# pbalcer/libpga

Measured on AMD Instinct MI355X. Metric: generations/sec + evals/sec, OneMax pop=1M 1024-bit, 1/2/4/8 MI355X, higher is better.
Workload: dtype u1-bitpacked; 1 GPU; model=OneMax-1024bit, global_batch=1048576, seq_len=1024, parallelism=island1, pop_per_gpu=1048576, selection=tournament-2, crossover=uniform, mutation=bit_flip, elitism=1, topology=ring, device=AMD Radeon Graphics

## Files before the change

csrc/include/pga/binary_dev.hpp:

```cpp
#pragma once
#include <hip/hip_runtime.h>

#include <type_traits>

#include "pga/device.hpp"
#include "pga/ops.hpp"
#include "pga/tp.hpp"

typedef __attribute__((address_space(3))) const unsigned int* pga_lds_words;
extern "C" __device__ float pga_user_objective(pga_lds_words words, unsigned int nbits, const float* data);

namespace pga {
#ifdef PGA_JIT_GEN
namespace jitgen {
#else
namespace {
#endif

using namespace dev;


template <int OBJ>
struct BinObj {
  uint32_t u = 0;
  uint32_t first0 = 0xFFFFFFFFu;
  float v = 0.f, w = 0.f;

  __device__ __forceinline__ void add(const GenArgs& a, uint4 x, uint32_t c) {
    const uint32_t wd[4] = {x.x, x.y, x.z, x.w};
    if (OBJ == OBJ_ONEMAX) {
      u += __popc(x.x) + __popc(x.y) + __popc(x.z) + __popc(x.w);
    } else if (OBJ == OBJ_KNAPSACK) {
      const float* val = a.obj_data;
      const float* wt = a.obj_data + a.L;
#pragma unroll
      for (int j = 0; j < 4; ++j) {
        uint32_t bits = wd[j];
        const uint32_t base = c * 128u + 32u * j;
        while (bits) {
          uint32_t b = __ffs(bits) - 1;
          bits &= bits - 1;
          v += val[base + b];
          w += wt[base + b];
        }
      }
    } else if (OBJ == OBJ_TRAP) {
      const uint32_t k = (uint32_t)a.obj_i;
      const uint32_t km = k >= 32 ? 0xFFFFFFFFu : ((1u << k) - 1u);
#pragma unroll
      for (int j = 0; j < 4; ++j) {
        const uint32_t base = c * 128u + 32u * j;
        for (uint32_t i = 0; i < 32u; i += k) {
          if (base + i + k > a.L) break;
          uint32_t ones = __popc((wd[j] >> i) & km);
          u += ones == k ? k : (k - 1 - ones);
        }
      }
    } else if (OBJ == OBJ_LEADING_ONES) {
#pragma unroll
      for (int j = 0; j < 4; ++j) {
        uint32_t inv = ~wd[j];
        if (inv != 0u) {
          uint32_t p = c * 128u + 32u * j + (__ffs(inv) - 1);
          first0 = p < first0 ? p : first0;
          break;
        }
      }
    }
  }

  template <int GS>
  __device__ __forceinline__ float finish(const GenArgs& a) {
    if (OBJ == OBJ_ONEMAX || OBJ == OBJ_TRAP) return (float)group_sum_u<GS>(u);
    if (OBJ == OBJ_KNAPSACK) {
      float vv = group_sum<GS>(v), ww = group_sum<GS>(w);
      return ww <= a.obj_f0 ? vv : a.obj_f0 - ww;
    }
    if (OBJ == OBJ_LEADING_ONES) {
      uint32_t m = group_min_u<GS>(first0);
      return (float)(m < a.L ? m : a.L);
    }
    return 0.f;
  }
};

__device__ __forceinline__ uint4 u4(u32x4 v) { return make_uint4(v.x, v.y, v.z, v.w); }
__device__ __forceinline__ uint4 and4(uint4 a, uint4 b) { return make_uint4(a.x & b.x, a.y & b.y, a.z & b.z, a.w & b.w); }
__device__ __forceinline__ uint4 xor4(uint4 a, uint4 b) { return make_uint4(a.x ^ b.x, a.y ^ b.y, a.z ^ b.z, a.w ^ b.w); }
__device__ __forceinline__ uint4 mix4(uint4 a, uint4 b, uint4 m) {
  return make_uint4((a.x & m.x) | (b.x & ~m.x), (a.y & m.y) | (b.y & ~m.y), (a.z & m.z) | (b.z & ~m.z),
                    (a.w & m.w) | (b.w & ~m.w));
}
__device__ __forceinline__ uint4 range_keep_a(uint32_t c, uint32_t lo, uint32_t hi) {
  const uint32_t b0 = c * 128u;
  return make_uint4(~range_mask32(b0, lo, hi), ~range_mask32(b0 + 32, lo, hi), ~range_mask32(b0 + 64, lo, hi),
                    ~range_mask32(b0 + 96, lo, hi));
}
__device__ __forceinline__ uint4 bit4(uint32_t b) {
  const uint32_t m = 1u << (b & 31u), j = b >> 5;
  return make_uint4(j == 0 ? m : 0u, j == 1 ? m : 0u, j == 2 ? m : 0u, j == 3 ? m : 0u);
}
__device__ __forceinline__ uint32_t chunk_len(uint32_t L, uint32_t c) {
  const uint32_t b = c * 128u;
  return L - b >= 128u ? 128u : L - b;
}

typedef int v4i __attribute__((ext_vector_type(4)));
constexpr int kObjKnapMfma = 1000;
constexpr uint32_t kKnapSlices = 8;
constexpr uint32_t kKnapMaxCols = 16;

__device__ __forceinline__ v4i expand16(uint32_t h) {
  v4i r;
  r[0] = (int)(__umul24(h & 0xFu, 0x00204081u) & 0x01010101u);
  r[1] = (int)(__umul24((h >> 4) & 0xFu, 0x00204081u) & 0x01010101u);
  r[2] = (int)(__umul24((h >> 8) & 0xFu, 0x00204081u) & 0x01010101u);
  r[3] = (int)(__umul24((h >> 12) & 0xFu, 0x00204081u) & 0x01010101u);
  return r;
}

__device__ __forceinline__ uint32_t knap_slot(uint32_t m, uint32_t h) { return 4u * m + (h ^ ((m >> 1) & 3u)); }
constexpr uint32_t kKnapCStride = 20;
constexpr uint32_t kKnapScratch = 16 * kKnapCStride / 4;

template <int GS>
__device__ __forceinline__ float knap_mfma(const GenArgs& a, uint4 v, uint32_t lane, uint32_t q, uint4* scr,
                                           const uint4* tab) {
  constexpr uint32_t R = GS / 4;
  const uint32_t D = a.knap_dig, NC = a.knap_cols;
  scr[knap_slot(lane >> 2, lane & 3u)] = v;
  wave_lds_sync();
  const uint32_t h = lane >> 4, n = lane & 15u;
  const uint4 x = scr[knap_slot(n, h)];
  const uint32_t xs[4] = {x.x, x.y, x.z, x.w};
  const uint4* tb = tab + h * kKnapMaxCols + n;
  v4i acc = {0, 0, 0, 0};
#pragma unroll
  for (uint32_t s = 0; s < kKnapSlices; ++s) {
    const uint4 t = tb[s * 4u * kKnapMaxCols];
    const uint32_t bits = (s & 1u) ? (xs[s >> 1] >> 16) : (xs[s >> 1] & 0xFFFFu);
    acc = __builtin_amdgcn_mfma_i32_16x16x64_i8(expand16(bits), v4i{(int)t.x, (int)t.y, (int)t.z, (int)t.w}, acc,
                                                0, 0, 0);
  }
  wave_lds_sync();
  int* cl = (int*)scr;
  *(v4i*)(cl + n * kKnapCStride + 4u * h) = acc;
  wave_lds_sync();
  const uint32_t g = lane / GS;
  uint32_t V = 0, W = 0;
  for (uint32_t e = q; e < NC; e += GS) {
    const uint32_t r = e / (2u * D), d = e % D;
    const uint32_t c = (uint32_t)cl[e * kKnapCStride + g * R + r] << (8u * d);
    if ((e / D) & 1u) W += c;
    else V += c;
  }
  const float vv = (float)(int)group_sum_u<GS>(V), ww = (float)(int)group_sum_u<GS>(W);
  return ww <= a.obj_f0 ? vv : a.obj_f0 - ww;
}

template <int GS, bool NH = false>
__device__ __forceinline__ uint4 sparse_continue(const GenArgs& a, uint64_t child, uint32_t K, uint32_t n, uint32_t j,
                                              uint4 fm, uint32_t q, uint32_t gbase) {
  u32x4 blk = draw<NH>(a.key, ST_BMUT, child, j >> 2);
  while (n < K) {
    if ((j & 3u) == 0u) blk = draw<NH>(a.key, ST_BMUT, child, j >> 2);
    const uint32_t p = word_to_index(sel4(blk, j & 3u), a.L);
    ++j;
    const uint32_t b = p & 127u;
    const bool own = (p >> 7) == q;
    const uint32_t wd = sel4(u32x4{fm.x, fm.y, fm.z, fm.w}, b >> 5);
    unsigned long long bal = __ballot(own && ((wd >> (b & 31u)) & 1u));
    if (GS < 64) bal = (bal >> gbase) & ((1ull << GS) - 1ull);
    if (bal == 0ull) {
      if (own) fm = xor4(fm, bit4(b));
      ++n;
    }
  }
  return fm;
}

template <bool NH>
__device__ __forceinline__ uint4 sparse_seq(const RngKey& key, uint64_t child, uint32_t kk, uint32_t L, uint32_t& jn) {
  uint32_t w0 = 0xFFFFFFFFu, w1 = 0xFFFFFFFFu, w2 = 0xFFFFFFFFu, w3 = 0xFFFFFFFFu;
  uint32_t n = 0, j = 0;
  u32x4 blk{0, 0, 0, 0};
  while (n < kk) {
    if ((j & 3u) == 0u) blk = draw<NH>(key, ST_BMUT, child, j >> 2);
    const uint32_t p = word_to_index(sel4(blk, j & 3u), L);
    ++j;
    const bool seen = (w0 & 0xFFFFu) == p || (w0 >> 16) == p || (w1 & 0xFFFFu) == p || (w1 >> 16) == p ||
                      (w2 & 0xFFFFu) == p || (w2 >> 16) == p || (w3 & 0xFFFFu) == p || (w3 >> 16) == p;
    if (!seen) {
      const uint32_t sh = (n & 1u) * 16u, keep = ~(0xFFFFu << sh), v = p << sh, wi = n >> 1;
      w0 = wi == 0u ? (w0 & keep) | v : w0;
      w1 = wi == 1u ? (w1 & keep) | v : w1;
      w2 = wi == 2u ? (w2 & keep) | v : w2;
      w3 = wi == 3u ? (w3 & keep) | v : w3;
      ++n;
    }
  }
  jn = j;
  return make_uint4(w0, w1, w2, w3);
}

template <int GS, int OBJ, int MODE>
__global__ __launch_bounds__(kBlock) void binary_kernel(GenArgs a, unsigned long long* best_parts) {
  resolve_gen(a);
  __shared__ unsigned long long lds_red[kBlock / 64];
  __shared__ uint32_t lds_elite;
  __shared__ uint32_t lds_thr[kMutCap];

  const uint32_t lane = lane_id();
  const uint32_t q = lane & (GS - 1);
  const uint32_t gbase = lane & ~(uint32_t)(GS - 1);
  constexpr uint32_t GPB = kBlock / GS;
  const uint32_t g_in_block = threadIdx.x / GS;
  const uint64_t rs = a.row_words >> 2;
  const uint4* cur = (const uint4*)a.cur;
  uint4* nxt = (uint4*)a.next;
  const uint32_t nchunks = a.chunks;
  const uint32_t L = a.L;
  constexpr bool MUTATES = MODE == MODE_GEN || MODE == MODE_MUTATE;
  constexpr bool EVALS = OBJ != OBJ_NONE && (MODE == MODE_GEN || MODE == MODE_INIT || MODE == MODE_EVAL);
  const bool bitflip = MUTATES && a.mutation == MUT_BIT_FLIP && a.mut_rate > 0.f;
  const bool sparse = bitflip && a.mut_sparse;
  const bool reset_one = MUTATES && a.mutation == MUT_RESET_ONE;

  if (MODE == MODE_GEN && a.n_elite > 0 && a.elite_idx == nullptr && blockIdx.x == 0) {
    unsigned long long b = block_reduce_parts(a.best_cur, a.n_best_cur, lds_red);
    if (threadIdx.x == 0) lds_elite = (uint32_t)best_index(b);
  }
  if (bitflip)
    for (uint32_t i = threadIdx.x; i < kMutCap; i += kBlock) lds_thr[i] = a.mut_thr[i];
  __syncthreads();

  unsigned long long my_best = 0;
  ScoreStats st;
  const uint64_t stride = (uint64_t)gridDim.x * GPB;
  for (uint64_t child = (uint64_t)blockIdx.x * GPB + g_in_block; child < a.S; child += stride) {
    float score = 0.f;
    {
      const bool elite = MODE == MODE_GEN && child < a.n_elite;
      uint32_t pa = 0, pb = 0;
      bool xo = false;
      uint32_t blo = 0, bhi = 0;
      u32x4 misc{0, 0, 0, 0};
      if (MODE == MODE_GEN || MODE == MODE_CROSS || MODE == MODE_MUTATE) misc = bin_misc(a.key, child);
      if (elite) {
        pa = pb = a.elite_idx ? a.elite_idx[child] : lds_elite;
      } else if (MODE == MODE_GEN || MODE == MODE_CROSS) {
        st_select_parents(a, child, pa, pb);
        xo = a.crossover != XO_NONE && do_crossover(a, misc.x);
        if (a.crossover == XO_ONE_POINT) {
          blo = word_to_index(misc.y, L);
          bhi = L;
        } else if (a.crossover == XO_TWO_POINT) {
          uint32_t c1 = word_to_index(misc.y, L);
          uint32_t c2 = word_to_index(misc.z, L);
          blo = c1 < c2 ? c1 : c2;
          bhi = c1 < c2 ? c2 : c1;
        }
      }
      uint32_t rpos = 0xFFFFFFFFu;
      if (reset_one && !elite && misc.w < a.mut_ind_thresh) rpos = word_to_index(bin_mut_word(a.key, child, 0), L);
      uint4 fm = make_uint4(0, 0, 0, 0);
      if (sparse && !elite) fm = sparse_continue<GS>(a, child, binom_count(misc.w, lds_thr), 0, 0, fm, q, gbase);

      BinObj<OBJ> acc;
      for (uint32_t c0 = 0; c0 < nchunks; c0 += GS) {
        const uint32_t c = c0 + q;
        if (c >= nchunks) continue;
        uint4 v = make_uint4(0, 0, 0, 0);
        if (MODE == MODE_INIT) {
          v = u4(draw(a.key, ST_INIT, child, c));
        } else if (MODE == MODE_EVAL || MODE == MODE_MUTATE) {
          v = cur[child * rs + c];
        } else {
          const uint4 A = cur[(uint64_t)pa * rs + c];
          if (xo) {
            const uint4 B = cur[(uint64_t)pb * rs + c];
            const uint4 m = a.crossover == XO_UNIFORM ? u4(draw(a.key, ST_XO, child, c)) : range_keep_a(c, blo, bhi);
            v = mix4(A, B, m);
          } else {
            v = A;
          }
        }
        if (c == nchunks - 1) v = and4(v, u4(a.last_mask));
        if (bitflip && !sparse && !elite) {
          v = xor4(v, u4(chunk_flip_mask(a, child, c, chunk_len(L, c), bin_chunk_mut_word(a.key, child, c), lds_thr)));
        } else if (sparse) {
          v = xor4(v, fm);
        } else if (reset_one && (rpos >> 7) == c) {
          v = xor4(v, bit4(rpos & 127u));
        }
        if (MODE != MODE_EVAL) nxt[child * rs + c] = v;
        if (EVALS) acc.add(a, v, c);
      }
      if (EVALS) score = acc.template finish<GS>(a);
    }
    if (EVALS && q == 0) {
      a.score_next[child] = score;
      if (a.key_next) a.key_next[child] = (uint16_t)score;
      const unsigned long long pb = pack_best(score, child);
      my_best = pb > my_best ? pb : my_best;
      st.add(score);
    }
  }
  if (EVALS && best_parts) {
    unsigned long long b = block_max_u64(my_best, lds_red);
    if (threadIdx.x == 0) best_parts[blockIdx.x] = b;
    if (a.stats_parts) block_stats_store(st, a.stats_parts);
  }
}


#ifdef PGA_TP_TIMING
__device__ unsigned long long pga_tp_clk[kMaxGrid * 4][8];
#endif


__device__ __forceinline__ uint32_t pos16(uint4 r1, uint32_t k) {
  const uint32_t w = sel4(u32x4{r1.x, r1.y, r1.z, r1.w}, k >> 1);
  return (k & 1u) ? (w >> 16) : (w & 0xFFFFu);
}

template <int GS, int OBJ, bool FULL, bool DENSE>
__device__ __forceinline__ void binary_gen_tp_body(GenArgs a, unsigned long long* best_parts) {
  resolve_gen(a);
  const uint32_t NW = blockDim.x >> 6;
  constexpr uint32_t NG = 64 / GS;
  constexpr uint32_t PD = tp_prefetch_depth(GS);
  constexpr bool EVALS = OBJ != OBJ_NONE;
  constexpr bool KEY = OBJ == OBJ_ONEMAX || OBJ == OBJ_LEADING_ONES || OBJ == OBJ_TRAP;
  uint4(*lds_rec)[2][64][2] = (uint4(*)[2][64][2])pga_dyn_lds;
  uint2* lds_par = (uint2*)(pga_dyn_lds + NW * 4096u);
  __shared__ uint32_t lds_thr[kMutCap];
  __shared__ uint32_t lds_el[kTpMaxElite];
  __shared__ unsigned long long lds_red[kTpMaxWaves];
  __shared__ uint32_t lds_next;
  __shared__ uint32_t lds_tnext;
  __shared__ uint32_t lds_ready[kTpMaxSegs];
  constexpr bool KMF = OBJ == kObjKnapMfma;
  __shared__ uint4 lds_kscr[KMF ? kTpMaxWaves : 1][kKnapScratch];
  __shared__ uint4 lds_ktab[KMF ? kKnapSlices * 4 * kKnapMaxCols : 1];
  constexpr bool JIT = OBJ == kObjJit;
  constexpr bool HISTK = KEY && !JIT;

  const uint32_t lane = lane_id(), wid = threadIdx.x >> 6;
  const uint32_t q = lane & (GS - 1), gbase = lane & ~(uint32_t)(GS - 1), g = lane / GS;
  const uint4* cur = (const uint4*)a.cur;
  uint4* nxt = (uint4*)a.next;
  const uint32_t L = a.L, S = (uint32_t)a.S;
  const bool have = FULL || q < a.chunks, last = q == a.chunks - 1;
  const uint32_t qq = have ? q : 0u;
  const uint32_t clen = have ? chunk_len(L, q) : 0u;
  const bool xo_on = a.crossover != XO_NONE;
  const bool range = a.crossover != XO_UNIFORM;
  const bool bitflip = a.mutation == MUT_BIT_FLIP && a.mut_rate > 0.f;
  const bool sparse = !DENSE && bitflip;
  const bool reset_one = !DENSE && a.mutation == MUT_RESET_ONE;
  const uint4 lmask = u4(a.last_mask);
  const uint32_t rb = a.row_words * 4u;
#define ELEM(T, base, i) (*(T*)((char*)(base) + (uint32_t)(i) * (uint32_t)sizeof(T)))
#define ROW(base, row, ch) (*(uint4*)((char*)(base) + ((uint32_t)(row) * rb + (uint32_t)(ch) * 16u)))

  const uint32_t U = tp_unit(a, NG);
  const uint32_t nst = U / NG;
  uint32_t bbegin, bend;
  tp_block_range(S, U, bbegin, bend, a.tp_skew);
  const uint32_t pcap = tp_par_cap(NW);
  uint4* lds_stage = (uint4*)(pga_dyn_lds + NW * 4096u + pcap * 8u) + wid * (kJitStageSteps * 64u);
  (void)lds_stage;
  uint32_t* lds_hist = (uint32_t*)(pga_dyn_lds + NW * 4096u + pcap * 8u);
  const bool hist = HISTK && (a.key_hist != nullptr || a.rank_counts != nullptr);
  const uint32_t hmax = a.hist_bins - 1u;

  __shared__ uint32_t lds_pro;
  bool pro_ok = false;
  if (KMF)
    for (uint32_t i = threadIdx.x; i < kKnapSlices * 4 * kKnapMaxCols; i += blockDim.x)
      lds_ktab[i] = ((const uint4*)a.knap_tab)[i];
  if (threadIdx.x == 0) lds_next = lds_tnext = lds_pro = 0;
  if (threadIdx.x < kTpMaxSegs) lds_ready[threadIdx.x] = 0;
  if (hist) {
    for (uint32_t i = threadIdx.x; i < a.hist_bins; i += blockDim.x) lds_hist[i] = 0;
    if (a.hist_zero)
      for (uint32_t i = blockIdx.x * blockDim.x + threadIdx.x; i < a.hist_zero_words; i += gridDim.x * blockDim.x)
        a.hist_zero[i] = 0;
  }

  unsigned long long my_best = 0;
  ScoreStats st;
  uint4(*rec)[64][2] = lds_rec[wid];
  static_assert(sizeof(lds_rec[0]) >= kSegBatches * 64 * sizeof(uint4), "contestant staging");
#ifdef PGA_TP_TIMING
  const unsigned long long clk0 = clock64(), rt0 = wall_clock64();
  unsigned long long clk_t = 0, clk_b = 0, n_bred = 0, clk_spin = 0;
#endif
  for (uint32_t rbeg = bbegin; rbeg < bend; rbeg += pcap) {
    const uint32_t rend = rbeg + pcap < bend ? rbeg + pcap : bend;
    const uint32_t nu = (rend - rbeg + U - 1) / U;
    const uint32_t nseg = (rend - rbeg + kSegBatches * 64 - 1) / (kSegBatches * 64);
    __syncthreads();
#ifdef PGA_TP_TIMING
    const unsigned long long clkA = clock64();
#endif
    if (rbeg == bbegin && wid == 0) {
      if (a.n_elite > 0 && bbegin < a.n_elite) {
        if (a.elite_idx) {
          for (uint32_t i = lane; i < a.n_elite; i += 64) lds_el[i] = a.elite_idx[i];
        } else {
          const unsigned long long b = wave_reduce_parts(a.best_cur, a.n_best_cur);
          if (lane == 0) lds_el[0] = (uint32_t)best_index(b);
        }
      }
      if (bitflip)
        for (uint32_t i = lane; i < kMutCap; i += 64) lds_thr[i] = a.mut_thr[i];
      __builtin_amdgcn_fence(__ATOMIC_RELEASE, "workgroup");
      tp_flag_set(&lds_pro);
    }

    for (;;) {
      const uint32_t sg = tp_ticket(&lds_tnext, lane);
      if (sg >= nseg) break;
      const uint32_t begin = rbeg + sg * kSegBatches * 64u;
      const uint32_t end = begin + kSegBatches * 64u < rend ? begin + kSegBatches * 64u : rend;
      uint2* par = lds_par + sg * kSegBatches * 64u;
      tp_select_segment<KEY ? TP_KEY16 : TP_F32>(a, begin, end, lane, &rec[0][0][0], par);
      __builtin_amdgcn_fence(__ATOMIC_RELEASE, "workgroup");
      tp_flag_set(&lds_ready[sg]);
    }
    if (NW < kTpMaxWaves) __syncthreads();
#ifdef PGA_TP_TIMING
    const unsigned long long clkB = clock64();
    clk_t += clkB - clkA;
#endif

#ifdef PGA_TP_TIMING
#define PGA_TP_SPIN0 const unsigned long long sp0_ = clock64();
#define PGA_TP_SPIN1 clk_spin += clock64() - sp0_;
#else
#define PGA_TP_SPIN0
#define PGA_TP_SPIN1
#endif
#define PGA_TP_RESOLVE(US, UE, SL)                                                                              \
  {                                                                                                             \
    if (!pro_ok) {                                           \
      while (__hip_atomic_load(&lds_pro, __ATOMIC_RELAXED, __HIP_MEMORY_SCOPE_WORKGROUP) == 0u)                 \
        __builtin_amdgcn_s_sleep(1);                                                                            \
      __builtin_amdgcn_fence(__ATOMIC_ACQUIRE, "workgroup");                                                    \
      pro_ok = true;                                                                                            \
    }                                                                                                           \
    const uint32_t tc = (US) + lane;                                                                            \
    const uint32_t cc = tc < (UE) ? tc : (UE) - 1;                                                              \
                                                             \
    const uint32_t sg_ = ((US) - rbeg) / (kSegBatches * 64u);                                                   \
    PGA_TP_SPIN0                                                                                                \
    while (__hip_atomic_load(&lds_ready[sg_], __ATOMIC_RELAXED, __HIP_MEMORY_SCOPE_WORKGROUP) == 0u)            \
      __builtin_amdgcn_s_sleep(1);                                                                              \
    PGA_TP_SPIN1                                                                                                \
    __builtin_amdgcn_fence(__ATOMIC_ACQUIRE, "workgroup");                                                      \
    const uint2 pp = lds_par[cc - rbeg];                              \
    uint32_t pa = pp.x, pb = pp.y;                                                                              \
    const u32x4 misc = bin_misc<true>(a.key, cc);                                                               \
    const bool elite = tc < a.n_elite;                                                                          \
    const bool xo = !elite && xo_on && do_crossover(a, misc.x);                                                 \
    if (elite) pa = lds_el[tc];                                                                                 \
    pb = xo ? pb : pa;                                                                                          \
    uint32_t lo = 0, hi = 0;                                                                                    \
    if (range && xo) {                                                                                          \
      const uint32_t x1 = word_to_index(misc.y, L);                                                             \
      if (a.crossover == XO_ONE_POINT) {                                                                        \
        lo = x1;                                                                                                \
        hi = L;                                                                                                 \
      } else {                                                                                                  \
        const uint32_t x2 = word_to_index(misc.z, L);                                                           \
        lo = x1 < x2 ? x1 : x2;                                                                                 \
        hi = x1 < x2 ? x2 : x1;                                                                                 \
      }                                                                                                         \
    }                                                                                                           \
    uint32_t K = 0, jn = 0;                                                                                     \
    uint4 P = make_uint4(0xFFFFFFFFu, 0xFFFFFFFFu, 0xFFFFFFFFu, 0xFFFFFFFFu);                                   \
    if (reset_one && !elite && misc.w < a.mut_ind_thresh) {                                                     \
      K = 1;                                                                                                    \
      P.x = word_to_index(bin_mut_word<true>(a.key, cc, 0), L) | 0xFFFF0000u;                                   \
    }                                                                                                           \
    if (sparse && !elite) {                                                                                     \
      K = binom_count(misc.w, lds_thr);                                                                         \
      if (K > 0u) {                                                                                             \
        const uint32_t kk = K < kRecPos ? K : kRecPos;                                                          \
        const u32x4 m0 = draw<true>(a.key, ST_BMUT, cc, 0);                                                     \
        const uint32_t c0 = word_to_index(m0.x, L), c1 = word_to_index(m0.y, L);                                \
        const uint32_t c2 = word_to_index(m0.z, L), c3 = word_to_index(m0.w, L);                                \
                              \
        const bool slow = kk > 4u || (kk > 1u && c0 == c1) || (kk > 2u && (c2 == c0 || c2 == c1)) ||            \
                          (kk > 3u && (c3 == c0 || c3 == c1 || c3 == c2));                                      \
        P = make_uint4(c0 | (c1 << 16), c2 | (c3 << 16), 0xFFFFFFFFu, 0xFFFFFFFFu);                             \
        jn = kk;                                                                                                \
        if (slow) P = sparse_seq<true>(a.key, cc, kk, L, jn);                                                   \
      }                                                                                                         \
    }                                                                                                           \
    const uint32_t meta = (K > 255u ? 255u : K) | ((jn > 0xFFFFu ? 0xFFFFu : jn) << 8) | (elite ? 1u << 31 : 0u); \
    uint4(*r)[2] = rec[(SL)];                                                                                   \
    r[lane][0] = make_uint4(pa, pb, lo | (hi << 16), meta);                                                     \
    r[lane][1] = P;                                                                                             \
  }

    constexpr uint32_t kNoUnit = 0xFFFFFFFFu;
#define PGA_TP_NEXT(US, UE)                                                                                 \
  {                                                                                                         \
    US = kNoUnit;                                                                                           \
    const uint32_t tk_ = tp_ticket(&lds_next, lane);                                                        \
    if (tk_ < nu) {                                                                                         \
      US = rbeg + tk_ * U;                                                                                  \
      UE = US + U < rend ? US + U : rend;                                                                   \
    }                                                                                                       \
  }

    uint32_t ns, ne = 0;
    PGA_TP_NEXT(ns, ne)
    if (ns != kNoUnit) {
      uint32_t slot = 0, i = 0, bs = ns, be = ne;
      PGA_TP_NEXT(ns, ne)
      PGA_TP_RESOLVE(bs, be, 0u)
      uint32_t lslot = 0, li = 0, lbs = bs, lbe = be;
      bool lpend = false, lmore = true, done = false;

#define PGA_TP_LOAD(YA, YB)                                                                                 \
  {                                                                                                         \
    if (lpend) {                                                                \
      PGA_TP_RESOLVE(ns, ne, lslot ^ 1u)                                                                    \
      lslot ^= 1u;                                                                                          \
      li = 0;                                                                                               \
      lbs = ns;                                                                                             \
      lbe = ne;                                                                                             \
      lpend = false;                                                                                        \
      PGA_TP_NEXT(ns, ne)                                                                                   \
    }                                                                                                       \
    const uint4 r = rec[lmore ? lslot : slot][(lmore ? li : i) * NG + g][0];                                \
    YA = ROW(cur, r.x, qq);                                                                                 \
    YB = ROW(cur, r.y, qq);                                                                                 \
    if (lmore && ++li == nst) {                                                                             \
      lpend = ns != kNoUnit;                                                                                \
      lmore = lpend;                                                                                        \
    }                                                                                                       \
  }

#define PGA_TP_STEP(XA, XB, YA, YB)                                                                         \
  {                                                                                                         \
    PGA_TP_LOAD(YA, YB)                                                                                     \
    const uint32_t c = bs + i * NG + g;                                                                     \
    const uint4 r0 = rec[slot][i * NG + g][0];                                                              \
    const uint32_t meta = r0.w;                                                                             \
    const uint4 m = range ? range_keep_a(q, r0.z & 0xFFFFu, r0.z >> 16) : u4(draw<true>(a.key, ST_XO, c, q)); \
    uint4 v = mix4(XA, XB, m);                                                                              \
    if (last) v = and4(v, lmask);                                                                           \
    uint4 fm = make_uint4(0, 0, 0, 0);                                                                      \
    if (DENSE) {                                                                                            \
      if (bitflip && !(meta >> 31))                                            \
        fm = u4(chunk_flip_mask(a, c, q, clen, bin_chunk_mut_word<true>(a.key, c, q), lds_thr));            \
    } else {                                                                                                \
      const uint32_t K = meta & 0xFFu;                                                                      \
      if (K > 0u) {                                                                                         \
        const uint4 r1 = rec[slot][i * NG + g][1];                                                          \
        const uint32_t kk = K < kRecPos ? K : kRecPos;                                                      \
                               \
        _Pragma("unroll") for (uint32_t k = 0; k < 4; ++k) {                                               \
          const uint32_t p = pos16(r1, k);                                                                  \
          if (k < kk && (p >> 7) == q) fm = xor4(fm, bit4(p & 127u));                                       \
        }                                                                                                   \
        if (kk > 4u)                                                                                        \
          for (uint32_t k = 4; k < kk; ++k) {                                                               \
            const uint32_t p = pos16(r1, k);                                                                \
            if ((p >> 7) == q) fm = xor4(fm, bit4(p & 127u));                                              \
          }                                                                                                 \
        if (K > kRecPos) fm = sparse_continue<GS, true>(a, c, K, kRecPos, (meta >> 8) & 0xFFFFu, fm, q, gbase); \
      }                                                                                                     \
    }                                                                                                       \
    v = xor4(v, fm);                                                                                        \
    float sc;                                                                                               \
    if constexpr (KMF) {                                                                                    \
      sc = knap_mfma<GS>(a, have ? v : make_uint4(0, 0, 0, 0), lane, q, lds_kscr[wid], lds_ktab);            \
    } else if constexpr (JIT) {                                                                             \
      sc = 0.f;                                                               \
    } else {                                                                                                \
      BinObj<OBJ> acc;                                                                                      \
      if (have) acc.add(a, v, q);                                                                           \
      sc = acc.template finish<GS>(a);                                                                      \
    }                                                                                                       \
    if (have) ROW(nxt, c, q) = v;                                                                           \
    if constexpr (JIT) {                                                                                    \
      lds_stage[(i % kJitStageSteps) * 64u + lane] = v;                                                     \
      if (i % kJitStageSteps == kJitStageSteps - 1u || i + 1u == nst) PGA_TP_JIT_EVAL                       \
    }                                                                                                       \
    if (EVALS && !JIT) {                                 \
      ELEM(float, a.score_next, c) = sc;                                                                    \
      if (KEY) ELEM(uint16_t, a.key_next, c) = (uint16_t)sc;                                                \
      if (hist && q == 0u && c < S) {                                                                       \
        const uint32_t kb = (uint16_t)sc;                                                                   \
        __hip_atomic_fetch_add(&lds_hist[kb < hmax ? kb : hmax], 1u, __ATOMIC_RELAXED,                      \
                               __HIP_MEMORY_SCOPE_WORKGROUP);                                               \
      }                                                                                                     \
      const unsigned long long pk = c < S ? pack_best(sc, c) : 0ull;                                        \
      my_best = pk > my_best ? pk : my_best;                                                                \
      st.add_if(q == 0u && c < S, sc);                                                                      \
    }                                                                                                       \
    if (++i == nst) {                                                                                       \
      PGA_TP_COUNT                                                                                          \
      if (lbs == bs) {                    \
        done = true;                                                                                        \
      } else {                                                                                              \
        slot ^= 1u;                                                                                         \
        i = 0;                                                                                              \
        bs = lbs;                                                                                           \
        be = lbe;                                                                                           \
      }                                                                                                     \
    }                                                                                                       \
  }

#define PGA_TP_JIT_EVAL                                                                                     \
  {                                                                                                         \
    __builtin_amdgcn_fence(__ATOMIC_RELEASE, "wavefront");                                                  \
    __builtin_amdgcn_fence(__ATOMIC_ACQUIRE, "wavefront");                                                  \
    const uint32_t s0 = i - i % kJitStageSteps, ns = i - s0 + 1u;                                           \
    const uint32_t cj = bs + s0 * NG + lane;                                                                \
    if (lane < ns * NG && cj < be) {                                                                        \
      const uint32_t js = lane / NG, jg = lane % NG;                                                        \
      const float sj = pga_user_objective((pga_lds_words)(lds_stage + js * 64u + jg * GS), L, a.obj_data);  \
      ELEM(float, a.score_next, cj) = sj;                                                                   \
      my_best = pack_best(sj, cj) > my_best ? pack_best(sj, cj) : my_best;                                  \
      st.add(sj);                                                                                           \
    }                                                                                                       \
    __builtin_amdgcn_fence(__ATOMIC_RELEASE, "wavefront");                                                  \
    __builtin_amdgcn_fence(__ATOMIC_ACQUIRE, "wavefront");                                                  \
  }
#ifdef PGA_TP_TIMING
#define PGA_TP_COUNT n_bred += be - bs;
#else
#define PGA_TP_COUNT
#endif

      uint4 A0, B0, A1, B1, A2, B2, A3, B3;
      (void)A2; (void)B2; (void)A3; (void)B3;
      if constexpr (PD == 1) {
        PGA_TP_LOAD(A0, B0)
        for (;;) {
          PGA_TP_STEP(A0, B0, A1, B1)
          if (done) break;
          PGA_TP_STEP(A1, B1, A0, B0)
          if (done) break;
        }
      } else if constexpr (PD == 2) {
        PGA_TP_LOAD(A0, B0)
        PGA_TP_LOAD(A1, B1)
        for (;;) {
          PGA_TP_STEP(A0, B0, A2, B2)
          if (done) break;
          PGA_TP_STEP(A1, B1, A0, B0)
          if (done) break;
          PGA_TP_STEP(A2, B2, A1, B1)
          if (done) break;
        }
      } else {
        PGA_TP_LOAD(A0, B0)
        PGA_TP_LOAD(A1, B1)
        PGA_TP_LOAD(A2, B2)
        for (;;) {
          PGA_TP_STEP(A0, B0, A3, B3)
          if (done) break;
          PGA_TP_STEP(A1, B1, A0, B0)
          if (done) break;
          PGA_TP_STEP(A2, B2, A1, B1)
          if (done) break;
          PGA_TP_STEP(A3, B3, A2, B2)
          if (done) break;
        }
      }
#undef PGA_TP_STEP
#undef PGA_TP_LOAD
#undef PGA_TP_NEXT
#undef PGA_TP_JIT_EVAL
#undef PGA_TP_COUNT
    }
#undef PGA_TP_RESOLVE
#undef PGA_TP_SPIN0
#undef PGA_TP_SPIN1
#ifdef PGA_TP_TIMING
    asm volatile("s_waitcnt vmcnt(0)" ::: "memory");
    clk_b += clock64() - clkB;
#endif
    __syncthreads();
    if (threadIdx.x == 0) lds_next = lds_tnext = 0;
    if (threadIdx.x < kTpMaxSegs) lds_ready[threadIdx.x] = 0;
  }
#undef ROW
#undef ELEM
#ifdef PGA_TP_TIMING
  if (lane == 0 && blockIdx.x * NW + wid < kMaxGrid * 4) {
    const uint32_t wv = blockIdx.x * NW + wid;
    pga_tp_clk[wv][0] = clk_t;
    pga_tp_clk[wv][1] = clk_b;
    pga_tp_clk[wv][2] = clock64() - clk0;
    pga_tp_clk[wv][3] = n_bred;
    pga_tp_clk[wv][4] = rt0;
    pga_tp_clk[wv][5] = wall_clock64();
    pga_tp_clk[wv][6] = __builtin_amdgcn_s_getreg((3 << 11) | 20);
    pga_tp_clk[wv][7] = clk_spin;
  }
#endif
  if (hist)
    for (uint32_t i = threadIdx.x; i < a.hist_bins; i += blockDim.x) {
      const uint32_t v = lds_hist[i];
      if (a.key_hist && v) __hip_atomic_fetch_add(&a.key_hist[i], v, __ATOMIC_RELAXED, __HIP_MEMORY_SCOPE_AGENT);
      if (a.rank_counts) a.rank_counts[i * gridDim.x + blockIdx.x] = v;
    }
  if (EVALS && best_parts) {
    unsigned long long bb = block_max_u64_n(my_best, lds_red, NW);
    if (threadIdx.x == 0) best_parts[blockIdx.x] = bb;
    if (a.stats_parts) block_stats_store_n(st, a.stats_parts, NW);
  }
}

template <int GS, int OBJ, bool FULL, bool DENSE>
__global__ __launch_bounds__(kTpMaxWaves * 64) void binary_gen_tp(GenArgs a, unsigned long long* best_parts) {
  binary_gen_tp_body<GS, OBJ, FULL, DENSE>(a, best_parts);
}

constexpr uint32_t kMaxBatch = 10;
struct GenBatch {
  GenArgs a[kMaxBatch];
  unsigned long long* parts[kMaxBatch];
};

template <int GS, int OBJ, bool FULL, bool DENSE>
__global__ __launch_bounds__(kTpMaxWaves * 64) void binary_gen_tp_batch(GenBatch b) {
  binary_gen_tp_body<GS, OBJ, FULL, DENSE>(b.a[blockIdx.y], b.parts[blockIdx.y]);
}

}
}
```

csrc/kernels/binary_gs.hip:

```cpp
#ifndef PGA_BIN_GS
#error "build with -DPGA_BIN_GS=<group size>"
#endif
#include <hip/hip_runtime.h>

#include <algorithm>
#include <cstdio>

#include "pga/device.hpp"
#include "pga/ops.hpp"
#include "pga/tp.hpp"
#include "pga/binary_dev.hpp"

namespace pga {
namespace {

using namespace dev;

template <typename K>
uint32_t go(K kernel, const GenArgs& a, unsigned long long* parts, uint32_t gpb, hipStream_t s) {
  const uint32_t grid = launch_grid_occ(a.S, gpb, (const void*)kernel);
  hipLaunchKernelGGL(kernel, grid, kBlock, 0, s, a, parts);
  return grid;
}

template <typename K>
uint32_t go_tp(K kernel, const GenArgs& a0, unsigned long long* parts, hipStream_t s) {
  const TpGeom t = tp_geometry(a0.S, 1, (const void*)kernel, 64 / group_size(a0.chunks));
  GenArgs a = a0;
  a.tp_unit = t.unit;
  a.tp_skew = tp_skew_units(t, a.S);
  const bool key_obj = a.objective == OBJ_ONEMAX || a.objective == OBJ_LEADING_ONES || a.objective == OBJ_TRAP;
  const bool hist = key_obj && a.key_cur != nullptr && a.key_hist != nullptr && a.hist_bins > 0 &&
                    a.hist_bins <= kHistMaxBins;
  if (!hist) a.key_hist = nullptr;
  const bool rk = key_obj && a.key_cur != nullptr && a.rank_counts != nullptr && a.hist_bins > 0 &&
                  a.hist_bins <= kHistMaxBins &&
                  (a.S + t.grid - 1) / t.grid == kRankTile && (uint64_t)t.grid == (a.S + kRankTile - 1) / kRankTile;
  if (rk) a.tp_skew = 0;
  else a.rank_counts = nullptr;
  hipLaunchKernelGGL(kernel, t.grid, t.block, t.lds + (hist || rk ? 4u * a.hist_bins : 0u), s, a, parts);
  binary_hist_written() = hist;
  binary_rank_counts_written() = rk;
  binary_tp_partition() = TpPartition{t.grid, tp_unit(a, 64u / group_size(a.chunks)), a.tp_skew};
  return t.grid;
}

template <int GS, int OBJ>
uint32_t launch_mode(int mode, const GenArgs& a, unsigned long long* parts, hipStream_t s) {
  constexpr uint32_t gpb = kBlock / GS;
  switch (mode) {
    case MODE_GEN: {
      const bool fast = a.chunks <= (uint32_t)GS &&
                        ((a.selection == SEL_TOURNAMENT && a.tour_k == 2) || a.selection == SEL_RANDOM ||
                         (a.selection == SEL_RANK && a.rank_order != nullptr) ||
                         (a.selection == SEL_ROULETTE && a.cumfit != nullptr && a.roul_guide != nullptr)) &&
                        !(a.n_elite > 1 && a.elite_idx == nullptr) && !force_generic_kernels();
      constexpr bool INT_OBJ = OBJ == OBJ_ONEMAX || OBJ == OBJ_LEADING_ONES || OBJ == OBJ_TRAP;
      const bool o32 = (a.S + kRowPad) * (uint64_t)a.row_words * 4u <= 0xFFFFFFFFull;
      if (fast && o32 && a.n_elite <= kTpMaxElite && (!INT_OBJ || a.key_cur != nullptr)) {
        if constexpr (OBJ == OBJ_KNAPSACK && GS >= 4 && GS <= 32) {
          if (a.knap_tab != nullptr &&
              (a.knap_cols == 0 || a.knap_cols > kKnapMaxCols || a.knap_dig == 0 || a.knap_dig > 4 ||
               a.knap_cols != (uint32_t)GS / 2u * a.knap_dig))
            throw std::invalid_argument("knapsack digit table does not match the genome geometry");
        }
        const bool dense = a.mutation == MUT_BIT_FLIP && a.mut_rate > 0.f && !a.mut_sparse;
        const bool full = a.chunks == (uint32_t)GS;
        if constexpr (OBJ == OBJ_KNAPSACK && GS >= 4 && GS <= 32) {
          if (a.knap_tab != nullptr) {
            if (full) {
              if (dense) return go_tp(binary_gen_tp<GS, kObjKnapMfma, true, true>, a, parts, s);
              return go_tp(binary_gen_tp<GS, kObjKnapMfma, true, false>, a, parts, s);
            }
            if (dense) return go_tp(binary_gen_tp<GS, kObjKnapMfma, false, true>, a, parts, s);
            return go_tp(binary_gen_tp<GS, kObjKnapMfma, false, false>, a, parts, s);
          }
        }
        if (full) {
          if (dense) return go_tp(binary_gen_tp<GS, OBJ, true, true>, a, parts, s);
          return go_tp(binary_gen_tp<GS, OBJ, true, false>, a, parts, s);
        }
        if (dense) return go_tp(binary_gen_tp<GS, OBJ, false, true>, a, parts, s);
        return go_tp(binary_gen_tp<GS, OBJ, false, false>, a, parts, s);
      }
      return go(binary_kernel<GS, OBJ, MODE_GEN>, a, parts, gpb, s);
    }
    case MODE_INIT: return go(binary_kernel<GS, OBJ, MODE_INIT>, a, parts, gpb, s);
    case MODE_EVAL: return go(binary_kernel<GS, OBJ, MODE_EVAL>, a, parts, gpb, s);
    case MODE_CROSS: return go(binary_kernel<GS, OBJ_NONE, MODE_CROSS>, a, parts, gpb, s);
    default: return go(binary_kernel<GS, OBJ_NONE, MODE_MUTATE>, a, parts, gpb, s);
  }
}

template <int GS>
uint32_t launch_obj(int mode, const GenArgs& a, unsigned long long* parts, hipStream_t s) {
  switch (a.objective) {
    case OBJ_ONEMAX: return launch_mode<GS, OBJ_ONEMAX>(mode, a, parts, s);
    case OBJ_KNAPSACK: return launch_mode<GS, OBJ_KNAPSACK>(mode, a, parts, s);
    case OBJ_TRAP: return launch_mode<GS, OBJ_TRAP>(mode, a, parts, s);
    case OBJ_LEADING_ONES: return launch_mode<GS, OBJ_LEADING_ONES>(mode, a, parts, s);
    default: return launch_mode<GS, OBJ_NONE>(mode, a, parts, s);
  }
}

}

template <>
uint32_t binary_launch_group<PGA_BIN_GS>(int mode, const GenArgs& a, unsigned long long* best_parts, hipStream_t s) {
  return launch_obj<PGA_BIN_GS>(mode, a, best_parts, s);
}

#if defined(PGA_TP_TIMING) && PGA_BIN_GS == 8
extern "C" void pga_tp_timing_dump(uint32_t nwaves) {
  static unsigned long long h[kMaxGrid * 4][8];
  PGA_HIP_CHECK(hipMemcpyFromSymbol(h, HIP_SYMBOL(pga_tp_clk), sizeof(h)));
  double t = 0, b = 0, tot = 0, n = 0, mx = 0;
  unsigned long long rt_min = ~0ull, rt_max = 0, st_max = 0;
  uint32_t nw = 0;
  for (uint32_t i = 0; i < nwaves && i < kMaxGrid * 4; ++i) {
    if (h[i][2] == 0) continue;
    t += (double)h[i][0];
    b += (double)h[i][1];
    tot += (double)h[i][2];
    mx = std::max(mx, (double)h[i][2]);
    n += 1;
    rt_min = std::min(rt_min, h[i][4]);
    rt_max = std::max(rt_max, h[i][5]);
    st_max = std::max(st_max, h[i][4]);
    nw = i + 1;
  }
  std::printf("{\"tp_timing\": {\"waves\": %.0f, \"tourn_cycles\": %.0f, \"breed_cycles\": %.0f, "
              "\"wave_cycles\": %.0f, \"max_wave_cycles\": %.0f, \"tourn_frac\": %.3f, "
              "\"span_us\": %.2f, \"last_start_us\": %.2f}}\n",
              n, t / n, b / n, tot / n, mx, t / (t + b), (rt_max - rt_min) / 100.0, (st_max - rt_min) / 100.0);
  double xe[8] = {0}, xm[8] = {0}, xn[8] = {0};
  const uint32_t bins = 8;
  double be[bins] = {0}, bm[bins] = {0}, bn[bins] = {0}, bs[bins] = {0};
  for (uint32_t i = 0; i < nw; ++i) {
    if (h[i][2] == 0) continue;
    const double e = (h[i][5] - rt_min) / 100.0, st = (h[i][4] - rt_min) / 100.0;
    const uint32_t x = (uint32_t)(h[i][6] & 7u), k = i * bins / nw;
    xe[x] += e; xn[x] += 1; xm[x] = std::max(xm[x], e);
    be[k] += e; bn[k] += 1; bm[k] = std::max(bm[k], e); bs[k] += st;
  }
  std::printf("{\"tp_xcd_end_us\": [");
  for (int x = 0; x < 8; ++x) std::printf("%s[%.1f, %.1f]", x ? ", " : "", xn[x] ? xe[x] / xn[x] : 0.0, xm[x]);
  std::printf("], \"tp_order_start_end_max_us\": [");
  for (uint32_t k = 0; k < bins; ++k)
    std::printf("%s[%.1f, %.1f, %.1f]", k ? ", " : "", bn[k] ? bs[k] / bn[k] : 0.0, bn[k] ? be[k] / bn[k] : 0.0, bm[k]);
  std::printf("]}\n");
}
#endif

}
```

Baseline: 11.64 billion evals/s.

## Add unit-fused breeding loop with shuffle-gathered scores and batched score stores

Adds a specialized breeding path for OneMax-style objectives with prefetch depth 2 and group size 4 or 8. It unrolls a whole 64-row unit with a rotating four-register prefetch across unit boundaries and gathers per-row scores into one lane each via shuffles. Each unit then issues one coalesced store of scores, keys, histogram, best and stats. This replaces scattered per-step score writes and per-step loop bookkeeping, at the cost of more registers, extra shuffles, and a tricky cross-unit prefetch index. It also adds barrier timing counters under the timing build flag.

```diff
diff --git a/csrc/include/pga/binary_dev.hpp b/csrc/include/pga/binary_dev.hpp
--- a/csrc/include/pga/binary_dev.hpp
+++ b/csrc/include/pga/binary_dev.hpp
@@ -315,7 +315,8 @@
 
 
 #ifdef PGA_TP_TIMING
-__device__ unsigned long long pga_tp_clk[kMaxGrid * 4][8];
+constexpr uint32_t kTpClkWords = 11;
+__device__ unsigned long long pga_tp_clk[kMaxGrid * 4][kTpClkWords];
 #endif
 
 
@@ -345,6 +346,7 @@
   __shared__ uint4 lds_ktab[KMF ? kKnapSlices * 4 * kKnapMaxCols : 1];
   constexpr bool JIT = OBJ == kObjJit;
   constexpr bool HISTK = KEY && !JIT;
+  constexpr bool UNITF = HISTK && PD == 2 && (GS == 4 || GS == 8);
 
   const uint32_t lane = lane_id(), wid = threadIdx.x >> 6;
   const uint32_t q = lane & (GS - 1), gbase = lane & ~(uint32_t)(GS - 1), g = lane / GS;
@@ -395,15 +397,20 @@
   static_assert(sizeof(lds_rec[0]) >= kSegBatches * 64 * sizeof(uint4), "contestant staging");
 #ifdef PGA_TP_TIMING
   const unsigned long long clk0 = clock64(), rt0 = wall_clock64();
-  unsigned long long clk_t = 0, clk_b = 0, n_bred = 0, clk_spin = 0;
+  unsigned long long clk_t = 0, clk_b = 0, n_bred = 0, clk_spin = 0, clk_sync0 = 0, clk_syncn = 0, clk_sync1 = 0;
 #endif
   for (uint32_t rbeg = bbegin; rbeg < bend; rbeg += pcap) {
     const uint32_t rend = rbeg + pcap < bend ? rbeg + pcap : bend;
     const uint32_t nu = (rend - rbeg + U - 1) / U;
     const uint32_t nseg = (rend - rbeg + kSegBatches * 64 - 1) / (kSegBatches * 64);
+#ifdef PGA_TP_TIMING
+    const unsigned long long clkS = clock64();
+#endif
     __syncthreads();
 #ifdef PGA_TP_TIMING
     const unsigned long long clkA = clock64();
+    if (rbeg == bbegin) clk_sync0 += clkA - clkS;
+    else clk_syncn += clkA - clkS;
 #endif
     if (rbeg == bbegin && wid == 0) {
       if (a.n_elite > 0 && bbegin < a.n_elite) {
@@ -546,11 +553,9 @@
     }                                                                                                       \
   }
 
-#define PGA_TP_STEP(XA, XB, YA, YB)                                                                         \
-  {                                                                                                         \
-    PGA_TP_LOAD(YA, YB)                                                                                     \
-    const uint32_t c = bs + i * NG + g;                                                                     \
-    const uint4 r0 = rec[slot][i * NG + g][0];                                                              \
+#define PGA_TP_BREED(XA, XB, I)                                                                             \
+    const uint32_t c = bs + (I) * NG + g;                                                                   \
+    const uint4 r0 = rec[slot][(I) * NG + g][0];                                                            \
     const uint32_t meta = r0.w;                                                                             \
     const uint4 m = range ? range_keep_a(q, r0.z & 0xFFFFu, r0.z >> 16) : u4(draw<true>(a.key, ST_XO, c, q)); \
     uint4 v = mix4(XA, XB, m);                                                                              \
@@ -562,7 +567,7 @@
     } else {                                                                                                \
       const uint32_t K = meta & 0xFFu;                                                                      \
       if (K > 0u) {                                                                                         \
-        const uint4 r1 = rec[slot][i * NG + g][1];                                                          \
+        const uint4 r1 = rec[slot][(I) * NG + g][1];                                                        \
         const uint32_t kk = K < kRecPos ? K : kRecPos;                                                      \
                                \
         _Pragma("unroll") for (uint32_t k = 0; k < 4; ++k) {                                               \
@@ -588,12 +593,10 @@
       if (have) acc.add(a, v, q);                                                                           \
       sc = acc.template finish<GS>(a);                                                                      \
     }                                                                                                       \
-    if (have) ROW(nxt, c, q) = v;                                                                           \
-    if constexpr (JIT) {                                                                                    \
-      lds_stage[(i % kJitStageSteps) * 64u + lane] = v;                                                     \
-      if (i % kJitStageSteps == kJitStageSteps - 1u || i + 1u == nst) PGA_TP_JIT_EVAL                       \
-    }                                                                                                       \
-    if (EVALS && !JIT) {                                 \
+    if (have) ROW(nxt, c, q) = v;
+
+#define PGA_TP_STEP_SCORE                                                                                   \
+    if (EVALS && !JIT) {                                                                                    \
       ELEM(float, a.score_next, c) = sc;                                                                    \
       if (KEY) ELEM(uint16_t, a.key_next, c) = (uint16_t)sc;                                                \
       if (hist && q == 0u && c < S) {                                                                       \
@@ -604,7 +607,17 @@
       const unsigned long long pk = c < S ? pack_best(sc, c) : 0ull;                                        \
       my_best = pk > my_best ? pk : my_best;                                                                \
       st.add_if(q == 0u && c < S, sc);                                                                      \
-    }                                                                                                       \
+    }
+
+#define PGA_TP_STEP(XA, XB, YA, YB)                                                                         \
+  {                                                                                                         \
+    PGA_TP_LOAD(YA, YB)                                                                                     \
+    PGA_TP_BREED(XA, XB, i)                                                                                 \
+    if constexpr (JIT) {                                                                                    \
+      lds_stage[(i % kJitStageSteps) * 64u + lane] = v;                                                     \
+      if (i % kJitStageSteps == kJitStageSteps - 1u || i + 1u == nst) PGA_TP_JIT_EVAL                       \
+    }                                                                                                       \
+    PGA_TP_STEP_SCORE                                                                                       \
     if (++i == nst) {                                                                                       \
       PGA_TP_COUNT                                                                                          \
       if (lbs == bs) {                    \
@@ -640,9 +653,76 @@
 #define PGA_TP_COUNT
 #endif
 
+#define PGA_TP_USTEP(I, XA, XB, YA, YB, NA, NB)                                                             \
+  {                                                                                                         \
+    const uint32_t ul_ = (I) + PD;                                                                          \
+    if (ul_ == (uint32_t)GS) {                         \
+      hn = ns != kNoUnit;                                                                                   \
+      if (hn) {                                                                                             \
+        PGA_TP_RESOLVE(ns, ne, slot ^ 1u)                                                                   \
+        nbs = ns;                                                                                           \
+        nbe = ne;                                                                                           \
+        PGA_TP_NEXT(ns, ne)                                                                                 \
+      }                                                                                                     \
+    }                                                                                                       \
+    const bool un_ = ul_ >= (uint32_t)GS;                                                                   \
+    const uint4 ur_ = rec[un_ && hn ? slot ^ 1u : slot][(un_ ? (hn ? ul_ - GS : (I)) : ul_) * NG + g][0];   \
+    YA = ROW(cur, ur_.x, qq);                                                                               \
+    YB = ROW(cur, ur_.y, qq);                                                                               \
+    {                                                                                                       \
+      const uint32_t w_ = NA.x | NB.x;                                                                      \
+      asm volatile("" ::"v"(w_));                                                                           \
+    }                                                                                                       \
+    PGA_TP_BREED(XA, XB, I)                                                                                 \
+    const float t_ = __shfl(sc, (int)usrc, 64);                                                             \
+    usc = lane / NG == (I) ? t_ : usc;                                                                      \
+  }
+
       uint4 A0, B0, A1, B1, A2, B2, A3, B3;
       (void)A2; (void)B2; (void)A3; (void)B3;
-      if constexpr (PD == 1) {
+      if (UNITF && U == 64u) {
+        float usc = 0.f;
+        const uint32_t usrc = (lane % NG) * GS + lane / NG;
+        bool hn = false;
+        uint32_t nbs = 0, nbe = 0;
+        {
+          const uint4 r = rec[0][g][0];
+          A0 = ROW(cur, r.x, qq);
+          B0 = ROW(cur, r.y, qq);
+        }
+        {
+          const uint4 r = rec[0][NG + g][0];
+          A1 = ROW(cur, r.x, qq);
+          B1 = ROW(cur, r.y, qq);
+        }
+        for (;;) {
+#pragma unroll
+          for (uint32_t u = 0; u < (uint32_t)GS; u += 4u) {
+            PGA_TP_USTEP(u, A0, B0, A2, B2, A1, B1)
+            PGA_TP_USTEP(u + 1u, A1, B1, A3, B3, A2, B2)
+            PGA_TP_USTEP(u + 2u, A2, B2, A0, B0, A3, B3)
+            PGA_TP_USTEP(u + 3u, A3, B3, A1, B1, A0, B0)
+          }
+          {
+            const uint32_t c = bs + lane;
+            ELEM(float, a.score_next, c) = usc;
+            ELEM(uint16_t, a.key_next, c) = (uint16_t)usc;
+            if (hist && c < S) {
+              const uint32_t kb = (uint16_t)usc;
+              __hip_atomic_fetch_add(&lds_hist[kb < hmax ? kb : hmax], 1u, __ATOMIC_RELAXED,
+                                     __HIP_MEMORY_SCOPE_WORKGROUP);
+            }
+            const unsigned long long pk = c < S ? pack_best(usc, c) : 0ull;
+            my_best = pk > my_best ? pk : my_best;
+            st.add_if(c < S, usc);
+          }
+          PGA_TP_COUNT
+          if (!hn) break;
+          slot ^= 1u;
+          bs = nbs;
+          be = nbe;
+        }
+      } else if constexpr (PD == 1) {
         PGA_TP_LOAD(A0, B0)
         for (;;) {
           PGA_TP_STEP(A0, B0, A1, B1)
@@ -676,7 +756,10 @@
           if (done) break;
         }
       }
+#undef PGA_TP_USTEP
 #undef PGA_TP_STEP
+#undef PGA_TP_STEP_SCORE
+#undef PGA_TP_BREED
 #undef PGA_TP_LOAD
 #undef PGA_TP_NEXT
 #undef PGA_TP_JIT_EVAL
@@ -687,9 +770,13 @@
 #undef PGA_TP_SPIN1
 #ifdef PGA_TP_TIMING
     asm volatile("s_waitcnt vmcnt(0)" ::: "memory");
-    clk_b += clock64() - clkB;
+    const unsigned long long clkE = clock64();
+    clk_b += clkE - clkB;
 #endif
     __syncthreads();
+#ifdef PGA_TP_TIMING
+    clk_sync1 += clock64() - clkE;
+#endif
     if (threadIdx.x == 0) lds_next = lds_tnext = 0;
     if (threadIdx.x < kTpMaxSegs) lds_ready[threadIdx.x] = 0;
   }
@@ -706,6 +793,9 @@
     pga_tp_clk[wv][5] = wall_clock64();
     pga_tp_clk[wv][6] = __builtin_amdgcn_s_getreg((3 << 11) | 20);
     pga_tp_clk[wv][7] = clk_spin;
+    pga_tp_clk[wv][8] = clk_sync0;
+    pga_tp_clk[wv][9] = clk_sync1;
+    pga_tp_clk[wv][10] = clk_syncn;
   }
 #endif
   if (hist)
diff --git a/csrc/kernels/binary_gs.hip b/csrc/kernels/binary_gs.hip
--- a/csrc/kernels/binary_gs.hip
+++ b/csrc/kernels/binary_gs.hip
@@ -112,9 +112,9 @@
 
 #if defined(PGA_TP_TIMING) && PGA_BIN_GS == 8
 extern "C" void pga_tp_timing_dump(uint32_t nwaves) {
-  static unsigned long long h[kMaxGrid * 4][8];
+  static unsigned long long h[kMaxGrid * 4][kTpClkWords];
   PGA_HIP_CHECK(hipMemcpyFromSymbol(h, HIP_SYMBOL(pga_tp_clk), sizeof(h)));
-  double t = 0, b = 0, tot = 0, n = 0, mx = 0;
+  double t = 0, b = 0, tot = 0, n = 0, mx = 0, s0 = 0, sn = 0, s1 = 0;
   unsigned long long rt_min = ~0ull, rt_max = 0, st_max = 0;
   uint32_t nw = 0;
   for (uint32_t i = 0; i < nwaves && i < kMaxGrid * 4; ++i) {
@@ -122,6 +122,9 @@
     t += (double)h[i][0];
     b += (double)h[i][1];
     tot += (double)h[i][2];
+    s0 += (double)h[i][8];
+    s1 += (double)h[i][9];
+    sn += (double)h[i][10];
     mx = std::max(mx, (double)h[i][2]);
     n += 1;
     rt_min = std::min(rt_min, h[i][4]);
@@ -130,9 +133,12 @@
     nw = i + 1;
   }
   std::printf("{\"tp_timing\": {\"waves\": %.0f, \"tourn_cycles\": %.0f, \"breed_cycles\": %.0f, "
+              "\"first_barrier_cycles\": %.0f, \"later_first_barrier_cycles\": %.0f, "
+              "\"last_barrier_cycles\": %.0f, "
               "\"wave_cycles\": %.0f, \"max_wave_cycles\": %.0f, \"tourn_frac\": %.3f, "
               "\"span_us\": %.2f, \"last_start_us\": %.2f}}\n",
-              n, t / n, b / n, tot / n, mx, t / (t + b), (rt_max - rt_min) / 100.0, (st_max - rt_min) / 100.0);
+              n, t / n, b / n, s0 / n, sn / n, s1 / n, tot / n, mx, t / (t + b), (rt_max - rt_min) / 100.0,
+              (st_max - rt_min) / 100.0);
   double xe[8] = {0}, xm[8] = {0}, xn[8] = {0};
   const uint32_t bins = 8;
   double be[bins] = {0}, bm[bins] = {0}, bn[bins] = {0}, bs[bins] = {0};
```

Result: faster. 12.03 billion evals/s (median of 6 runs) (+3.4%).
